# zkonduit/ezkl

Measured on AMD Instinct MI355X. Metric: BN254 G1 MSM pts/s (2^20 points per GPU; NTT 2^22 elems/s in extra), higher is better.
Workload: dtype u32x8 (254-bit modular integer, Montgomery); 1 GPU; configs[1]: standalone 2^20-point BN254 G1 MSM (uniform scalars, try-and-increment bases) + 2^22 scalar-field NTT per GPU; parallelism=points sharded across 1 rank(s); all_gather of 64-B partials + host fold

## Files before the change

ezkl_amd/csrc/msm.hip:

```cpp
#include "common.hpp"
#include <deque>
#include <thread>
#include <chrono>
#include "curve.hpp"
#include "curve29.hpp"
#include "host64.hpp"
#include "msm_plan.hpp"
#include <string.h>

namespace ezkl {

__device__ __forceinline__ uint32_t msm_part_of(uint32_t bucket, uint32_t NP) { return bucket ? 1u + (bucket & (NP - 1u)) : 0u; }
__device__ __forceinline__ uint32_t msm_lane_len(const uint32_t* offsets, uint32_t nb, uint32_t nlanes, uint32_t lmin) {
    const uint32_t l = (uint32_t)(((uint64_t)offsets[nb] + nlanes - 1) / nlanes);
    return l < lmin ? lmin : l;
}

template <class T> __device__ __forceinline__ T* bshift(T* p, size_t bytes) { return reinterpret_cast<T*>(reinterpret_cast<char*>(p) + bytes); }
template <class T> __device__ __forceinline__ const T* bshift(const T* p, size_t bytes) {
    return reinterpret_cast<const T*>(reinterpret_cast<const char*>(p) + bytes);
}
#define BSH(p) p = bshift(p, _bo)
#define BOFF() const size_t _bo = (size_t)blockIdx.z * bstride
struct MsmCols {
// ... 453 lines not shown
            const uint32_t e = beg + t + (uint32_t)q * 512u;
            v[q] = e < end ? entries[e] : make_uint2(0u, 0xffffffffu);
        }
#pragma unroll
        for (int q = 0; q < PER; q++)
            if (v[q].y != 0xffffffffu) atomicAdd(&cnt[v[q].y], 1u);
        __syncthreads();
        msm_bins_scan(cnt, tsum, nbins, p, beg, part_base, true, offsets, buckets);
#pragma unroll
        for (int q = 0; q < PER; q++)
            if (v[q].y != 0xffffffffu) stage[atomicAdd(&cnt[v[q].y], 1u)] = v[q].x;
        __syncthreads();
        for (uint32_t i = t; i < end - beg; i += 512) vals[beg + i] = stage[i];
    } else {
        for (uint32_t e = beg + t; e < end; e += 512) (void)msm_wave_rank(cnt, entries[e].y);
        __syncthreads();
        msm_bins_scan(cnt, tsum, nbins, p, beg, part_base, true, offsets, buckets);
        for (uint32_t e = beg + t; e < end; e += 512) {
            const uint2 v = entries[e];
            vals[beg + msm_wave_rank(cnt, v.y)] = v.x;
        }
    }
}
__device__ __forceinline__ void msm_big_slice(uint32_t beg, uint32_t end, uint32_t& s0, uint32_t& s1, uint32_t bx) {
    const uint32_t chunk = (end - beg + MSM_BIG_BLOCKS - 1) / MSM_BIG_BLOCKS;
    s0 = beg + bx * chunk;
    s1 = s0 + chunk < end ? s0 + chunk : end;
    if (s0 > end) s0 = end;
}
__device__ __forceinline__ void msm_bigsort_count_body(const uint2* entries, const uint32_t* part_base, uint32_t LB, const uint32_t* big_list,
                                                       const uint32_t* big_count, uint32_t* bin_total, uint32_t* block_off, uint32_t* cnt, uint32_t bx,
                                                       uint32_t by, uint32_t rows) {
    const uint32_t t = threadIdx.x, nbins = 1u << LB;
    const uint32_t nbig = big_count[0] < MSM_MAX_BIG ? big_count[0] : MSM_MAX_BIG;
    for (uint32_t y = by; y < nbig; y += rows) {
        const uint32_t p = big_list[y];
        uint32_t s0, s1;
        msm_big_slice(part_base[p + 1], part_base[p + 2], s0, s1, bx);
        for (uint32_t j = t; j < nbins; j += 512) cnt[j] = 0;
        __syncthreads();
        for (uint32_t e = s0 + t; e < s1; e += 512) (void)msm_wave_rank(cnt, entries[e].y);
        __syncthreads();
        for (uint32_t j = t; j < nbins; j += 512)
            block_off[((size_t)y * MSM_BIG_BLOCKS + bx) * nbins + j] = cnt[j] ? atomicAdd(&bin_total[(size_t)y * nbins + j], cnt[j]) : 0u;
        __syncthreads();
    }
}
__global__ __launch_bounds__(512) void msm_bigsort_scatter_kernel(const uint2* entries, const uint32_t* part_base, uint32_t LB, const uint32_t* big_list,
                                                                  const uint32_t* big_count, const uint32_t* bin_total, const uint32_t* block_off,
                                                                  uint32_t* offsets, uint32_t* vals, g1x29_t* buckets, size_t bstride) {
    BOFF(); BSH(entries); BSH(part_base); BSH(big_list); BSH(big_count); BSH(bin_total); BSH(block_off); BSH(offsets); BSH(vals); BSH(buckets);
    __shared__ uint32_t cnt[2048];
    __shared__ uint32_t tsum[512];
    const uint32_t t = threadIdx.x, nbins = 1u << LB;
    const uint32_t nbig = big_count[0] < MSM_MAX_BIG ? big_count[0] : MSM_MAX_BIG;
    for (uint32_t y = blockIdx.y; y < nbig; y += gridDim.y) {
        const uint32_t p = big_list[y], beg = part_base[p + 1];
        uint32_t s0, s1;
        msm_big_slice(beg, part_base[p + 2], s0, s1, blockIdx.x);
        for (uint32_t j = t; j < nbins; j += 512) cnt[j] = bin_total[(size_t)y * nbins + j];
        __syncthreads();
        msm_bins_scan(cnt, tsum, nbins, p, beg, part_base, blockIdx.x == 0, offsets, buckets);
        const uint32_t* mine = block_off + ((size_t)y * MSM_BIG_BLOCKS + blockIdx.x) * nbins;
        for (uint32_t j = t; j < nbins; j += 512) atomicAdd(&cnt[j], mine[j]);
        __syncthreads();
        for (uint32_t e = s0 + t; e < s1; e += 512) {
            const uint2 v = entries[e];
            vals[beg + msm_wave_rank(cnt, v.y)] = v.x;
        }
        __syncthreads();
    }
}

struct MsmRec {
    g1a_t p;
    bool neg;
};
__device__ __forceinline__ MsmRec msm_fetch(const g1a_t* tab, uint32_t v) {
    MsmRec r;
    r.p = ld_g1a(tab + (v & 0x7fffffffu));
    r.neg = (v >> 31) != 0;
    return r;
}
__global__ __launch_bounds__(256, 3) void msm_accumulate_kernel(const g1a_t* tab, const uint32_t* offsets, const uint32_t* vals,
                                                             uint32_t nb, uint32_t nlanes, g1x29_t* buckets, g1x29_t* head, g1x29_t* tail,
                                                             uint32_t* lane_first, uint32_t lmin, size_t bstride) {
    BOFF(); BSH(offsets); BSH(vals); BSH(buckets); BSH(head); BSH(tail); BSH(lane_first);
    const uint32_t t = blockIdx.x * blockDim.x + threadIdx.x;
    const uint32_t total = offsets[nb], L = msm_lane_len(offsets, nb, nlanes, lmin);
    const uint64_t k0w = (uint64_t)t * L;
    if (k0w >= total) return;
    const uint32_t k0 = (uint32_t)k0w;
    const uint32_t k1 = (uint64_t)k0 + L < total ? k0 + L : total;
    uint32_t lo = 0, hi = nb;
    while (hi - lo > 1) {
        uint32_t mid = (lo + hi) >> 1;
        if (offsets[mid] <= k0) lo = mid; else hi = mid;
    }
    uint32_t b = lo, bin_end = offsets[b + 1];
    uint32_t end_next = offsets[b + 2 <= nb ? b + 2 : nb];
    lane_first[t] = b;
    bool started_before = offsets[b] < k0;
    g1x29_t acc = g1x29_identity();
    MsmRec nxt = msm_fetch(tab, vals[k0]);
    uint32_t vn = k0 + 1 < k1 ? vals[k0 + 1] : 0u;
    for (uint32_t k = k0; k < k1; k++) {
        if (k == bin_end) {
            if (started_before) st_g1x29(head + t, acc); else st_g1x29(buckets + b, acc);
            acc.zz = Fq29::zero();
            started_before = false;
            b++;
            bin_end = end_next;
            if (bin_end == k) {
                uint32_t probes = 1;
                while (bin_end == k && probes < 4) { b++; bin_end = offsets[b + 1]; probes++; }
                if (bin_end == k) {
                    uint32_t lo2 = b + 1, hi2 = nb, vhi = total;
                    while (hi2 - lo2 > 1) {
                        const uint32_t mid = (lo2 + hi2) >> 1, vm = offsets[mid];
                        if (vm <= k) lo2 = mid; else { hi2 = mid; vhi = vm; }
                    }
                    b = lo2;
                    bin_end = vhi;
                }
            }
        }
        end_next = offsets[b + 2 <= nb ? b + 2 : nb];
        const MsmRec cur = nxt;
        nxt = msm_fetch(tab, vn);
        vn = k + 2 < k1 ? vals[k + 2] : 0u;
        acc = g1x29_add_mixed(acc, g1a29_unpack(cur.p), cur.neg);
    }
    if (k1 == bin_end) {
        if (started_before) st_g1x29(head + t, acc); else st_g1x29(buckets + b, acc);
    } else {
        if (started_before) st_g1x29(head + t, acc); else st_g1x29(tail + t, acc);
    }
}
EZ_D g1x29_t g1x29_shfl_down(const g1x29_t& p, uint32_t d) {
    g1x29_t r;
    const uint32_t* s = p.x.v;
    uint32_t* o = r.x.v;
#pragma unroll
    for (int k = 0; k < 36; k++) o[k] = __shfl_down(s[k], d);
    return r;
}
__global__ __launch_bounds__(256, 3) void msm_fixup_boundary_tree_kernel(const uint32_t* offsets, uint32_t nb, uint32_t nlanes,
                                                                      const uint32_t* lane_first, const g1x29_t* head, const g1x29_t* tail, g1x29_t* buckets,
                                                                      uint32_t* heavy_list, uint32_t* heavy_count, uint32_t* chunk_list, uint32_t lmin,
                                                                      uint32_t span_heavy, size_t bstride) {
    BOFF(); BSH(offsets); BSH(lane_first); BSH(head); BSH(tail); BSH(buckets); BSH(heavy_list); BSH(heavy_count); BSH(chunk_list);
    const uint32_t t = blockIdx.x * blockDim.x + threadIdx.x + 1;
    const uint32_t lane = threadIdx.x & 63u;
    const uint32_t L = msm_lane_len(offsets, nb, nlanes, lmin);
    const uint64_t k0 = (uint64_t)t * L;
    bool cut = t < nlanes && k0 < offsets[nb];
    uint32_t b = 0, t1 = 0, t2 = 0;
    if (cut) {
        b = lane_first[t];
        const uint32_t beg = offsets[b], end = offsets[b + 1];
        cut = beg < k0;
        t1 = beg / L; t2 = (end - 1) / L;
    }
    if (cut && t2 - t1 > span_heavy) {
        if (t == t1 + 1 && t2 - t1 > MSM_HEAVY_CHUNK) heavy_list[atomicAdd(heavy_count, 1u)] = b;
        if ((t - t1 - 1) % MSM_HEAVY_CHUNK == 0) chunk_list[atomicAdd(heavy_count + 1, 1u)] = t;
        cut = false;
    }
    const uint32_t wave_last = t + (63u - lane);
    const uint32_t run = cut ? (t2 < wave_last ? t2 : wave_last) - t + 1u : 0u;
    uint32_t longest = run;
#pragma unroll
    for (uint32_t o = 32; o > 0; o >>= 1) {
        const uint32_t m = __shfl_xor(longest, o);
        longest = m > longest ? m : longest;
    }
    if (longest == 0) return;
    if (longest <= 2) {
        if (!cut || t != t1 + 1) return;
        g1x29_t acc = g1x29_add(ld_g1x29(tail + t1), ld_g1x29(head + t));
        for (uint32_t u = t + 1; u <= t2; u++) acc = g1x29_add(acc, ld_g1x29(head + u));
        st_g1x29(buckets + b, acc);
        return;
    }
    g1x29_t v = cut ? ld_g1x29(head + t) : g1x29_identity();
    uint32_t have = cut ? 1u : 0u;
#pragma unroll 1
    for (uint32_t d = 1; d < longest; d <<= 1) {
        const g1x29_t w = g1x29_shfl_down(v, d);
        const uint32_t hw = __shfl_down(have, d);
        if (have == d && run > d) {
            v = g1x29_add(v, w);
            have += hw;
        }
    }
    if (!cut || t != t1 + 1) return;
    g1x29_t acc = g1x29_add(ld_g1x29(tail + t1), v);
    for (uint32_t u = t + run; u <= t2; u++) acc = g1x29_add(acc, ld_g1x29(head + u));
    st_g1x29(buckets + b, acc);
}
__global__ __launch_bounds__(256) void msm_fixup_heavy1_kernel(const uint32_t* offsets, uint32_t nb, uint32_t nlanes, const uint32_t* lane_first, g1x29_t* head,
                                                               const g1x29_t* tail, g1x29_t* buckets, const uint32_t* chunk_list, const uint32_t* counts, uint32_t lmin,
                                                               uint32_t coop, size_t bstride) {
    BOFF(); BSH(offsets); BSH(lane_first); BSH(head); BSH(tail); BSH(buckets); BSH(chunk_list); BSH(counts);
    const uint32_t nchunks = counts[1], L = msm_lane_len(offsets, nb, nlanes, lmin);
    const uint32_t wave = threadIdx.x >> 6, lane = threadIdx.x & 63u;
    for (uint32_t ci = blockIdx.x * 4u + wave; ci < nchunks; ci += gridDim.x * 4u) {
        const uint32_t start = chunk_list[ci], b = lane_first[start];
        const uint32_t t2 = (offsets[b + 1] - 1) / L;
        const uint32_t stop = start + MSM_HEAVY_CHUNK - 1 < t2 ? start + MSM_HEAVY_CHUNK - 1 : t2;
        const uint32_t t1 = offsets[b] / L;
        const bool whole = t2 - t1 <= MSM_HEAVY_CHUNK;
        g1x29_t acc = (whole && lane == 63u) ? ld_g1x29(tail + t1) : g1x29_identity();
        for (uint32_t t = start + lane; t <= stop; t += 64) acc = g1x29_add(acc, ld_g1x29(head + t));
        acc = coop ? g1x29_group_sum_coop(acc, 64) : g1x29_group_sum(acc, 64);
        if (lane == 0) st_g1x29(whole ? buckets + b : head + start, acc);
    }
}
__global__ __launch_bounds__(256) void msm_fixup_heavy2_kernel(const uint32_t* offsets, uint32_t nb, uint32_t nlanes, const g1x29_t* head, const g1x29_t* tail,
                                                               const uint32_t* heavy_list, const uint32_t* counts, g1x29_t* buckets, uint32_t lmin, uint32_t coop, size_t bstride) {
    BOFF(); BSH(offsets); BSH(head); BSH(tail); BSH(heavy_list); BSH(counts); BSH(buckets);
    const uint32_t L = msm_lane_len(offsets, nb, nlanes, lmin);
    const uint32_t wave = threadIdx.x >> 6, lane = threadIdx.x & 63u;
    for (uint32_t h = blockIdx.x * 4u + wave; h < counts[0]; h += gridDim.x * 4u) {
        const uint32_t b = heavy_list[h];
        const uint32_t t1 = offsets[b] / L, t2 = (offsets[b + 1] - 1) / L;
        g1x29_t acc = lane == 63u ? ld_g1x29(tail + t1) : g1x29_identity();
        for (uint32_t t = t1 + 1 + lane * MSM_HEAVY_CHUNK; t <= t2; t += 64 * MSM_HEAVY_CHUNK) acc = g1x29_add(acc, ld_g1x29(head + t));
        acc = coop ? g1x29_group_sum_coop(acc, 64) : g1x29_group_sum(acc, 64);
        if (lane == 0) st_g1x29(buckets + b, acc);
    }
}

__global__ __launch_bounds__(256, 2) void msm_reduce1_kernel(const g1x29_t* buckets, ReduceGeom g, g1x29_t* partA, g1x29_t* partT, size_t bstride) {
    BOFF(); BSH(buckets); BSH(partA); BSH(partT);
    const uint32_t idx = blockIdx.x * blockDim.x + threadIdx.x;
    g1x29_t acc = g1x29_identity();
    if (blockIdx.y == 0) {
        if (idx >= (g.GA << g.wA)) return;
        const uint32_t dA = idx & ((1u << g.wA) - 1u), grp = idx >> g.wA;
        for (uint32_t e = 0; e < g.EA; e++) acc = g1x29_add(acc, ld_g1x29(buckets + ((((size_t)grp * g.EA + e) << g.wA) | dA)));
        st_g1x29(partA + (size_t)dA * g.GA + grp, acc);
    } else {
        const uint32_t nT = 1u << (g.wB + g.wC);
        if (idx >= nT * g.GT) return;
        const uint32_t grp = idx % g.GT, t = idx / g.GT;
        for (uint32_t e = 0; e < g.ET; e++) acc = g1x29_add(acc, ld_g1x29(buckets + (((size_t)t << g.wA) | (e * g.GT + grp))));
        st_g1x29(partT + (size_t)t * g.GT + grp, acc);
    }
}
__global__ __launch_bounds__(64) void msm_reduce2_kernel(const g1x29_t* partA, const g1x29_t* partT, ReduceGeom g, g1x29_t* SA, g1x29_t* T, uint32_t lanesA,
                                                         uint32_t lanesT, uint32_t blocksA, uint32_t coop, size_t bstride) {
    BOFF(); BSH(partA); BSH(partT); BSH(SA); BSH(T);
    const bool isA = blockIdx.x < blocksA;
    const uint32_t lanes = isA ? lanesA : lanesT, per = 64 / lanes;
    const uint32_t o = (isA ? blockIdx.x : blockIdx.x - blocksA) * per + threadIdx.x / lanes, j = threadIdx.x % lanes;
    const uint32_t nout = isA ? (1u << g.wA) : (1u << (g.wB + g.wC)), G = isA ? g.GA : g.GT;
    g1x29_t acc = g1x29_identity();
    if (o < nout) {
        const g1x29_t* src = (isA ? partA : partT) + (size_t)o * G;
        for (uint32_t i = j; i < G; i += lanes) acc = g1x29_add(acc, ld_g1x29(src + i));
    }
    acc = (coop && lanes >= 4) ? g1x29_group_sum_coop(acc, lanes) : g1x29_group_sum(acc, lanes);
    if (j == 0 && o < nout) st_g1x29((isA ? SA : T) + o, acc);
}
__global__ __launch_bounds__(256) void msm_planes_kernel(const g1x29_t* SA, const g1x29_t* T, ReduceGeom g, g1x29_t* planes, g1x29_t* planes_host, uint32_t coop,
                                                         size_t bstride) {
    BOFF(); BSH(SA); BSH(T); BSH(planes);
    __shared__ uint4 sh[9 * 4];
    uint32_t id = blockIdx.x, field = 0, j = 0;
    if (id > 0) {
        id -= 1;
        if (id < g.wA) { field = 1; j = id; }
        else if (id < g.wA + g.wB) { field = 2; j = id - g.wA; }
        else { field = 3; j = id - g.wA - g.wB; }
    }
    const uint32_t nA = 1u << g.wA, nT = 1u << (g.wB + g.wC);
    g1x29_t acc = g1x29_identity();
    auto with_bit = [](uint32_t k, uint32_t bit) { return ((k >> bit) << (bit + 1)) | (1u << bit) | (k & ((1u << bit) - 1u)); };
    if (field == 0) {
        for (uint32_t d = threadIdx.x; d < nA; d += 256) acc = g1x29_add(acc, ld_g1x29(SA + d));
    } else if (field == 1) {
        for (uint32_t k = threadIdx.x; k < nA / 2; k += 256) acc = g1x29_add(acc, ld_g1x29(SA + with_bit(k, j)));
    } else {
        const uint32_t sh_bits = field == 2 ? j : g.wB + j;
        for (uint32_t k = threadIdx.x; k < nT / 2; k += 256) acc = g1x29_add(acc, ld_g1x29(T + with_bit(k, sh_bits)));
    }
    acc = (coop & 8u) ? g1x29_block256_sum_coop_full(acc, sh) : coop ? g1x29_block256_sum_coop(acc, sh) : g1x29_block256_sum(acc, sh);
    if (threadIdx.x == 0) {
        const uint32_t ws = field == 1 ? g.wsA : field == 2 ? g.wsB : g.wsC;
        const uint32_t slot = field == 0 ? 0u : 1u + ws + j;
        st_g1x29(planes + slot, acc);
        if (planes_host) st_g1x29(planes_host + (size_t)blockIdx.z * 32 + slot, acc);
    }
}

static int table_build(Ctx* c, hipStream_t st, const Bases* b, bool wait) {
    MsmTable t;
    t.n = b->n;
    t.wp = pick_plan(b->n);
    if ((size_t)t.wp.W * t.n >= ((size_t)1 << 31)) return EZKL_ERR_UNSUPPORTED;
    EZ_HIP(hipMalloc(&t.tab, (size_t)t.wp.W * t.n * sizeof(g1a_t)));
    EZ_HIP(hipMemcpyAsync(t.tab, b->pts, t.n * sizeof(g1a_t), hipMemcpyDeviceToDevice, st));
    for (uint32_t w = 1; w < t.wp.W; w++)
        hipLaunchKernelGGL(msm_precompute_kernel, dim3(cdiv(t.n, 256)), dim3(256), 0, st, t.tab + (size_t)(w - 1) * t.n,
                           t.tab + (size_t)w * t.n, t.n, t.wp.width(w - 1));
    hipLaunchKernelGGL(msm_table_to_r261_kernel, dim3(cdiv((size_t)t.wp.W * t.n, 256)), dim3(256), 0, st, t.tab, (size_t)t.wp.W * t.n);
    EZ_HIP(hipGetLastError());
    EZ_HIP(hipEventCreateWithFlags(&t.ready, hipEventDisableTiming));
    EZ_HIP(hipEventRecord(t.ready, st));
    if (wait) {
        EZ_HIP(hipStreamSynchronize(st));
        t.synced = true;
    }
    g_tables[b] = t;
    return EZKL_OK;
}
static int table_get(Ctx* c, hipStream_t st, const Bases* b, MsmTable** out) {
    auto it = g_tables.find(b);
    if (it == g_tables.end()) {
        int rc = table_build(c, st, b, true);
        if (rc) return rc;
        it = g_tables.find(b);
    }
    if (!it->second.synced) {
        EZ_HIP(hipEventSynchronize(it->second.ready));
        it->second.synced = true;
    }
    *out = &it->second;
    return EZKL_OK;
}
int msm_table_prepare(Ctx* c, const Bases* b) {
    if (g_tables.count(b)) return EZKL_OK;
    if (!g_table_stream) EZ_HIP(hipStreamCreateWithFlags(&g_table_stream, hipStreamNonBlocking));
    return table_build(c, g_table_stream, b, false);
}
void msm_table_drop(const Bases* b) {
    auto it = g_tables.find(b);
    if (it != g_tables.end()) {
        if (it->second.ready) { (void)hipEventSynchronize(it->second.ready); (void)hipEventDestroy(it->second.ready); }
        (void)hipFree(it->second.tab);
        g_tables.erase(it);
    }
}

static int slot_prepare(MsmSlot& sl, size_t bytes, size_t msms = 1) {
    if (!sl.st) {
        EZ_HIP(stream_create_prio(&sl.st, "EZKL_HIP_PRIO_MSM", 0));
        EZ_HIP(hipEventCreateWithFlags(&sl.done, hipEventDisableTiming));
    }
    if (msms > sl.pinned_msms) {
        if (sl.pinned) {
            EZ_HIP(hipStreamSynchronize(sl.st));
            EZ_HIP(hipHostFree(sl.pinned));
            sl.pinned = nullptr;
        }
        EZ_HIP(hipHostMalloc((void**)&sl.pinned, msms * 32 * sizeof(g1x29_t), hipHostMallocDefault));
        EZ_HIP(hipHostGetDevicePointer(&sl.pinned_dev, sl.pinned, 0));
        sl.pinned_msms = msms;
    }
    if (bytes > sl.scratch_bytes) {
        if (sl.scratch) {
            EZ_HIP(hipStreamSynchronize(sl.st));
            EZ_HIP(hipFree(sl.scratch));
            sl.scratch = nullptr;
            sl.scratch_bytes = 0;
        }
        size_t want = bytes + (bytes >> 4);
        EZ_HIP(hipMalloc((void**)&sl.scratch, want));
        sl.scratch_bytes = want;
    }
    return EZKL_OK;
}
static int msm_finish(MsmSlot& sl, void* out_host = nullptr, bool release = true) {
    if (!out_host) out_host = sl.out;
    EZ_HIP(hipEventSynchronize(sl.done));
    for (uint32_t j = 0; j < sl.count; j++) {
        const uint32_t* hp = sl.pinned + (size_t)j * 32 * 36;
        h64::xyzz acc = h64::identity();
        for (int k = (int)sl.bits - 1; k >= 0; k--) {
            acc = h64::dbl(acc);
            acc = h64::add(acc, h64::from_limbs29_point(hp + 36 * (1 + k)));
        }
        acc = h64::add(acc, h64::from_limbs29_point(hp));
        h64::aff r = h64::to_affine(acc);
        memcpy((uint8_t*)out_host + 64 * (size_t)j, &r, 64);
    }
    if (release) sl.busy = false;
    return EZKL_OK;
}

struct MsmKnobs : MsmTuning {
    int group, group_small, group_big;
};
static int msm_env(const char* name, int hi, int dflt) { const char* e = getenv(name); const int v = e ? atoi(e) : 0; return v >= 1 && v <= hi ? v : dflt; }
static MsmKnobs msm_tuning() {
    static const int lmin = msm_env("EZKL_MSM_LMIN", 4096, (int)MSM_LMIN), span = msm_env("EZKL_MSM_SPAN", 4096, (int)MSM_SPAN_HEAVY);
    static const int small = msm_env("EZKL_MSM_GROUP_SMALL", (int)MSM_MAX_GROUP, 6), big = msm_env("EZKL_MSM_GROUP_BIG", (int)MSM_MAX_GROUP, 4);
    MsmKnobs k;
    k.lmin = (uint32_t)lmin; k.span_heavy = (uint32_t)span; k.group_small = small; k.group_big = big;
    k.L_override = (uint32_t)msm_env("EZKL_MSM_L", (1 << 20) - 1, 0);
    const int e = msm_env("EZKL_MSM_E", 1024, 0);
    if (e && (e & (e - 1)) == 0) k.E = (uint32_t)e;
    k.group = msm_env("EZKL_MSM_GROUP", (int)MSM_MAX_GROUP, 0);
    return k;
}
static size_t msm_group_size(bool small_scalars) {
    const MsmKnobs k = msm_tuning();
    return (size_t)(k.group ? k.group : small_scalars ? k.group_small : k.group_big);
}
static int msm_device_init(int& acc_blocks_per_cu) {
    if (acc_blocks_per_cu) return EZKL_OK;
    EZ_HIP(hipFuncSetAttribute((const void*)msm_binsort_kernel, hipFuncAttributeMaxDynamicSharedMemorySize, MSM_BINSORT_LDS));
    EZ_HIP(hipFuncSetAttribute((const void*)msm_partition_kernel, hipFuncAttributeMaxDynamicSharedMemorySize, MSM_PART_LDS));
    EZ_HIP(hipOccupancyMaxActiveBlocksPerMultiprocessor(&acc_blocks_per_cu, msm_accumulate_kernel, 256, 0));
    if (acc_blocks_per_cu < 1) acc_blocks_per_cu = 1;
    return EZKL_OK;
}
static_assert(sizeof(g1x29_t) == MSM_POINT_BYTES, "msm_plan lays the scratch out in points of this size");
static int msm_enqueue(Ctx* c, MsmSlot& sl, hipStream_t st, MsmTable* T, size_t base_offset, const fe_t* const* cols, size_t count, size_t n, bool timed) {
    int rc = EZKL_OK;
    if (count < 1 || count > MSM_MAX_GROUP) return EZKL_ERR_INVALID;
    const unsigned Z = (unsigned)count;
    const MsmKnobs tu = msm_tuning();
    int& acc_blocks_per_cu = msm_state().acc_blocks_per_cu;
    if ((rc = msm_device_init(acc_blocks_per_cu))) return rc;
    const MsmPlan p = msm_plan(n, T->wp, count, c->num_cus, acc_blocks_per_cu, tu);
    const WinPlan wp = T->wp;
    const ReduceGeom rg = p.rg;
    const uint32_t nb = p.nb, LB = p.LB, NP = p.NP, NQ = p.NQ, nlanes = p.nlanes, lmin = tu.lmin, span_heavy = tu.span_heavy;
    const size_t per_block = p.per_block, bstride = p.bstride;
    constexpr uint32_t coop = 7;
    rc = slot_prepare(sl, p.slab_bytes * count, count);
    if (rc) return rc;
    uint8_t* S = sl.scratch;
    MsmCols kcols;
    for (size_t j = 0; j < MSM_MAX_GROUP; j++) kcols.col[j] = cols[j < count ? j : 0];
    auto u32 = [&](size_t o) { return (uint32_t*)(S + o); };
    auto pt = [&](size_t o) { return (g1x29_t*)(S + o); };
    uint2* entries = (uint2*)(S + p.o.ent);
    uint32_t *vals = u32(p.o.vals), *offs = u32(p.o.offs), *pcnt = u32(p.o.pcnt), *pbase = u32(p.o.pbase), *wghist = u32(p.o.wghist);
    uint32_t *heavy = u32(p.o.heavy), *hcnt = u32(p.o.hcnt), *chunks = u32(p.o.chunks), *lfirst = u32(p.o.lfirst);
    uint32_t *bflag = u32(p.o.bflag), *blist = u32(p.o.blist), *btot = u32(p.o.btot), *boff = u32(p.o.boff);
    uint32_t* bcnt = hcnt + 2;
    g1x29_t *bkt = pt(p.o.bkt), *head = pt(p.o.head), *tail = pt(p.o.tail), *planes = pt(p.o.planes);
    g1x29_t *partA = pt(p.o.partA), *partT = pt(p.o.partT), *SA = pt(p.o.SA), *TT = pt(p.o.T);

    hipEvent_t m0 = nullptr, m1 = nullptr, a0 = nullptr, a1 = nullptr;
    bool timed_chain = timed;
    if (timed) {
        const char* tm = getenv("EZKL_HIP_TIMING");
        if (tm && !strcmp(tm, "none")) timed = timed_chain = false;
        else if (tm && !strcmp(tm, "kernel")) timed_chain = false;
    }
    if (timed) {
        if (timed_chain && (rc = ev_pair(c, "msm", &m0, &m1))) return rc;
        if ((rc = ev_pair(c, "msm_accumulate", &a0, &a1))) return rc;
        if (timed_chain) EZ_HIP(hipEventRecord(m0, st));
    }
    hipLaunchKernelGGL(msm_hist_kernel, dim3(p.sgrid, 1, Z), dim3(256), 0, st, kcols, n, per_block, wp, LB, NP, wghist, hcnt,
                       (uint32_t)(p.zero_bytes / 4), bstride);
    hipLaunchKernelGGL(msm_hist_scan_kernel, dim3(cdiv(NQ, MSM_SCAN_COLS), 1, Z), dim3(1024), 0, st, wghist, p.sgrid, NQ, pcnt, bstride);
    hipLaunchKernelGGL(msm_part_scan_kernel, dim3(1, 1, Z), dim3(1024), 0, st, pcnt, NQ, pbase, bflag, blist, bcnt, bstride);
    hipLaunchKernelGGL(msm_partition_kernel, dim3(p.pgrid, 1, Z), dim3((unsigned)per_block), p.part_lds, st, kcols, n, per_block,
                       (uint32_t)p.sgrid, wp, LB, NP, base_offset, T->n, pbase, wghist, pcnt, entries, vals, bstride);
    hipLaunchKernelGGL(msm_binsort_kernel, dim3(NP + MSM_BIG_BLOCKS * MSM_BIG_ROWS, 1, Z), dim3(512), MSM_BINSORT_STAGE * 4, st, entries, pbase, LB, NP, bflag, offs,
                       vals, bkt, blist, bcnt, btot, boff, bstride);
    hipLaunchKernelGGL(msm_bigsort_scatter_kernel, dim3(MSM_BIG_BLOCKS, MSM_BIG_ROWS, Z), dim3(512), 0, st, entries, pbase, LB, blist, bcnt, btot, boff, offs,
                       vals, bkt, bstride);
    if (timed) EZ_HIP(hipEventRecord(a0, st));
    hipLaunchKernelGGL(msm_accumulate_kernel, dim3(cdiv(nlanes, 256), 1, Z), dim3(256), 0, st, T->tab, offs, vals, nb, nlanes, bkt, head, tail,
                       lfirst, lmin, bstride);
    if (timed) EZ_HIP(hipEventRecord(a1, st));
    if (nlanes > 1)
        hipLaunchKernelGGL(msm_fixup_boundary_tree_kernel, dim3(cdiv(nlanes - 1, 256), 1, Z), dim3(256), 0, st, offs, nb, nlanes, lfirst, head, tail, bkt,
                           heavy, hcnt, chunks, lmin, span_heavy, bstride);
    hipLaunchKernelGGL(msm_fixup_heavy1_kernel, dim3(p.cb, 1, Z), dim3(256), 0, st, offs, nb, nlanes, lfirst, head, tail, bkt, chunks, hcnt, lmin, coop & 4u, bstride);
    hipLaunchKernelGGL(msm_fixup_heavy2_kernel, dim3(p.hb, 1, Z), dim3(256), 0, st, offs, nb, nlanes, head, tail, heavy, hcnt, bkt, lmin, coop & 4u, bstride);
    hipLaunchKernelGGL(msm_reduce1_kernel, dim3(p.r1grid, 2, Z), dim3(256), 0, st, bkt, rg, partA, partT, bstride);
    hipLaunchKernelGGL(msm_reduce2_kernel, dim3(p.r2grid, 1, Z), dim3(64), 0, st, partA, partT, rg, SA, TT, p.lanesA, p.lanesT, p.blocksA, coop & 1u, bstride);
    hipLaunchKernelGGL(msm_planes_kernel, dim3(p.nplanes, 1, Z), dim3(256), 0, st, SA, TT, rg, planes, (g1x29_t*)sl.pinned_dev, coop & 10u, bstride);
    EZ_HIP(hipGetLastError());
    if (getenv("EZKL_MSM_DEBUG")) {
        uint32_t hc = 0;
        EZ_HIP(hipMemcpyAsync(&hc, hcnt, 4, hipMemcpyDeviceToHost, st));
        EZ_HIP(hipStreamSynchronize(st));
        fprintf(stderr, "[msm] n=%zu W=%u bits=%u L=%u nlanes=%u heavy=%u\n", n, p.W, p.bits, p.L, nlanes, hc);
    }
    if (timed_chain) EZ_HIP(hipEventRecord(m1, st));
    EZ_HIP(hipEventRecord(sl.done, st));
    sl.bits = p.bits;
    sl.count = (uint32_t)count;
    sl.busy = true;
    return EZKL_OK;
}
static int msm_run_groups(Ctx* c, MsmTable* T, size_t base_offset, const fe_t* const* cols, size_t batch, size_t n, void* out_host,
                          const hipEvent_t* wait_ev, bool small_scalars) {
    const size_t G = msm_group_size(small_scalars);
    static const bool dbg = getenv("EZKL_MSM_DEBUG") != nullptr;
    if (dbg) fprintf(stderr, "[ezkl_hip] msm batch: %zu columns of %zu points, %s scalars, groups of %zu\n", batch, n, small_scalars ? "witness-shaped" : "general", G);
    int rc = EZKL_OK;
    size_t gi = 0;
    for (size_t j0 = 0; j0 < batch && !rc; gi++) {
        size_t cnt = batch - j0 < G ? batch - j0 : G;
        if (wait_ev && j0 > 0) {
            const size_t left = batch - j0;
            cnt = left <= 2 ? 1 : std::min(G, (left + 1) / 2);
        }
        MsmSlot& sl = g_slots[gi % MSM_SLOTS];
        if (sl.busy) rc = msm_finish(sl);
        if (!rc) rc = slot_prepare(sl, 0);
        for (size_t j = 0; wait_ev && j < cnt && !rc; j++)
            if (hipStreamWaitEvent(sl.st, wait_ev[j0 + j], 0) != hipSuccess) rc = EZKL_ERR_HIP;
        if (!rc) {
            sl.out = (uint8_t*)out_host + 64 * j0;
            rc = msm_enqueue(c, sl, sl.st, T, base_offset, cols + j0, cnt, n, false);
        }
        j0 += cnt;
    }
    for (size_t k = 0; k < (size_t)MSM_SLOTS; k++) {
        MsmSlot& sl = g_slots[(gi + k) % MSM_SLOTS];
        if (!sl.busy) continue;
        if (!rc) rc = msm_finish(sl);
        else { (void)hipStreamSynchronize(sl.st); sl.busy = false; }
    }
    return rc;
}

static bool msm_host_timing() { static const bool on = getenv("EZKL_MSM_HOST_TIMING") != nullptr; return on; }
static double msm_now_us() { return std::chrono::duration<double, std::micro>(std::chrono::steady_clock::now().time_since_epoch()).count(); }
static void msm_host_timing_add(size_t n, double t0, double t1, double t2, double t3) {
    static double acc[3] = {0, 0, 0};
    static int calls = 0;
    acc[0] += t1 - t0; acc[1] += t2 - t1; acc[2] += t3 - t2;
    if (++calls % 50 == 0) {
        fprintf(stderr, "[msm host] n=%zu per call: enqueue %.1f us, wait for the GPU %.1f us, host tail %.1f us\n", n, acc[0] / 50, acc[1] / 50, acc[2] / 50);
        acc[0] = acc[1] = acc[2] = 0;
    }
}
static MsmBatch* g_open_batch_fwd();
int msm_run(Ctx* c, hipStream_t st, const Bases* b, size_t base_offset, const fe_t* scalars, size_t n, void* out_host) {
    if (g_open_batch_fwd()) return EZKL_ERR_INVALID;
    if (n == 0) { memset(out_host, 0, 64); return EZKL_OK; }
    MsmTable* T = nullptr;
    int rc = table_get(c, st, b, &T);
    if (rc) return rc;
    MsmSlot& sl = g_slots[0];
    if (sl.busy) return EZKL_ERR_INVALID;
    const bool host_timing = msm_host_timing();
    const double t0 = host_timing ? msm_now_us() : 0;
    if ((rc = msm_enqueue(c, sl, st, T, base_offset, &scalars, 1, n, true))) return rc;
    if (!host_timing) return msm_finish(sl, out_host);
    const double t1 = msm_now_us();
    EZ_HIP(hipEventSynchronize(sl.done));
    const double t2 = msm_now_us();
    rc = msm_finish(sl, out_host);
    msm_host_timing_add(n, t0, t1, t2, msm_now_us());
    return rc;
}

int msm_call_start(Ctx* c, std::unique_lock<std::recursive_mutex>& lk, const Bases* b, size_t base_offset, const fe_t* scalars, size_t n, int* slot_out) {
    if (g_open_batch_fwd() || n == 0) return EZKL_ERR_INVALID;
    MsmTable* T = nullptr;
    int rc = table_get(c, c->stream, b, &T);
    if (rc) return rc;
    int k = -1;
    for (;;) {
        for (int i = 0; i < MSM_CALL_SLOTS && k < 0; i++)
            if (!g_call_claimed[i]) k = i;
        if (k >= 0) break;
        bool all_mine = true;
        for (int i = 0; i < MSM_CALL_SLOTS; i++) all_mine = all_mine && g_call_owner[i] == std::this_thread::get_id();
        if (all_mine) return EZKL_ERR_BUSY;
        lk.unlock();
        std::this_thread::yield();
        lk.lock();
    }
    MsmSlot& sl = g_call_slots[k];
    g_call_claimed[k] = true;
    g_call_finishing[k] = false;
    g_call_owner[k] = std::this_thread::get_id();
    rc = slot_prepare(sl, 0);
    if (!rc) {
        hipError_t e = hipSuccess;
        const hipError_t q = hipStreamQuery(c->stream);
        if (q != hipSuccess) {
            (void)hipGetLastError();
            if (!g_call_order_ev) e = hipEventCreateWithFlags(&g_call_order_ev, hipEventDisableTiming);
            if (e == hipSuccess) e = hipEventRecord(g_call_order_ev, c->stream);
            if (e == hipSuccess) e = hipStreamWaitEvent(sl.st, g_call_order_ev, 0);
        }
        if (e != hipSuccess) rc = set_hip_error(e, "msm_call_start", __FILE__, __LINE__);
    }
    if (!rc) rc = msm_enqueue(c, sl, sl.st, T, base_offset, &scalars, 1, n, true);
    if (rc) { g_call_claimed[k] = false; g_call_owner[k] = std::thread::id(); return rc; }
    *slot_out = k;
    return EZKL_OK;
}
int msm_call_finish(Ctx* c, std::unique_lock<std::recursive_mutex>& lk, int k, void* out_host) {
    (void)c;
    if (k < 0 || k >= MSM_CALL_SLOTS || !g_call_claimed[k] || g_call_finishing[k] || !g_call_slots[k].busy) return EZKL_ERR_INVALID;
    MsmSlot& sl = g_call_slots[k];
    g_call_finishing[k] = true;
    lk.unlock();
    const int rc = msm_finish(sl, out_host, false);
    lk.lock();
    sl.busy = false;
    g_call_finishing[k] = false;
    g_call_claimed[k] = false;
    g_call_owner[k] = std::thread::id();
    return rc;
}
int msm_run_concurrent(Ctx* c, std::unique_lock<std::recursive_mutex>& lk, const Bases* b, size_t base_offset, const fe_t* scalars, size_t n, void* out_host) {
    if (g_open_batch_fwd()) return EZKL_ERR_INVALID;
    if (n == 0) { memset(out_host, 0, 64); return EZKL_OK; }
    int k = -1;
    const bool host_timing = msm_host_timing();
    const double t0 = host_timing ? msm_now_us() : 0;
    int rc = msm_call_start(c, lk, b, base_offset, scalars, n, &k);
    if (rc) return rc;
    if (!host_timing) return msm_call_finish(c, lk, k, out_host);
    const double t1 = msm_now_us();
    (void)hipEventSynchronize(g_call_slots[k].done);
    const double t2 = msm_now_us();
    rc = msm_call_finish(c, lk, k, out_host);
    msm_host_timing_add(n, t0, t1, t2, msm_now_us());
    return rc;
}

int msm_run_batch(Ctx* c, hipStream_t st, const Bases* b, size_t base_offset, const fe_t* const* scalars, size_t batch, size_t n,
                  void* out_host, bool small_scalars) {
// ... 351 lines not shown
```

ezkl_amd/csrc/msm_plan.hpp:

```cpp
#pragma once
#include <cstddef>
#include <cstdint>
#if defined(__HIPCC__) || defined(__HIP__)
#define MSM_HD __host__ __device__
#else
#define MSM_HD
#endif

namespace ezkl {

static constexpr uint32_t MSM_MAX_PART_BITS = 12;
static constexpr uint32_t MSM_SPAN_HEAVY = 16;
static constexpr uint32_t MSM_PART_STAGE = 13312;
static constexpr uint32_t MSM_BINSORT_STAGE = 15360;
static constexpr uint32_t MSM_HEAVY_CHUNK = 256;
static constexpr uint32_t MSM_DIGIT_E = 8;
static constexpr uint32_t MSM_LMIN = 8;
static constexpr uint32_t MSM_MAX_BIG = 64;
static constexpr uint32_t MSM_BIG_BLOCKS = 64;
static constexpr uint32_t MSM_BIG_ROWS = 8;
static constexpr uint32_t MSM_SCAN_COLS = 4;
static constexpr size_t MSM_MAX_GROUP = 16;
static constexpr uint32_t MSM_PART_LDS = 144u << 10;
static constexpr uint32_t MSM_BINSORT_LDS = 96u << 10;
static constexpr size_t MSM_POINT_BYTES = 144;

struct WinPlan {
    uint32_t W, base, rem;
    MSM_HD uint32_t width(uint32_t w) const { return base + (w < rem ? 1u : 0u); }
    MSM_HD uint32_t offset(uint32_t w) const { return w * base + (w < rem ? w : rem); }
    MSM_HD uint32_t cmax() const { return base + (rem ? 1u : 0u); }
};
inline WinPlan pick_plan(size_t n) {
    WinPlan best{0, 0, 0};
    double best_cost = 0;
    for (uint32_t W = 10; W <= 127; W++) {
        WinPlan p{W, 254 / W, 254 % W};
        if (p.cmax() > 23) continue;
        const double cost = (double)n * W + 4.0 * (double)((size_t)1 << (p.cmax() - 1));
        if (!best.W || cost < best_cost) { best = p; best_cost = cost; }
    }
    return best;
}

struct ReduceGeom {
    uint32_t wA, wB, wC;
    uint32_t wsA, wsB, wsC;
    uint32_t EA, GA, ET, GT;
};

struct MsmTuning {
    uint32_t L_override = 0;
    uint32_t E = MSM_DIGIT_E;
    uint32_t lmin = MSM_LMIN;
    uint32_t span_heavy = MSM_SPAN_HEAVY;
};

struct MsmPlan {
    uint32_t W, bits, nb, PB, LB, NP, NQ, L, nlanes;
    size_t npairs, per_block, part_lds;
    unsigned sgrid, pgrid, hb, cb, r1grid, r2grid;
    ReduceGeom rg;
    uint32_t nA, nT, n_partA, n_partT, nplanes, lanesA, lanesT, blocksA;
    struct Off { size_t ent, vals, offs, pcnt, pbase, wghist, heavy, chunks, hcnt, btot, planes, bflag, blist, boff, lfirst, bkt, head, tail, partA, partT, SA, T; } o;
    size_t zero_bytes, slab_bytes, bstride;
};

inline MsmPlan msm_plan(size_t n, WinPlan wp, size_t count, int num_cus, int acc_blocks_per_cu, const MsmTuning& tu) {
    MsmPlan p{};
    auto cdiv = [](size_t a, size_t b) { return (unsigned)((a + b - 1) / b); };
    const uint32_t W = p.W = wp.W, bits = p.bits = wp.cmax() - 1;
    const uint32_t nb = p.nb = 1u << bits;
    const size_t npairs = p.npairs = n * W;
    uint32_t PB = bits < 10 ? bits : 10;
    while (PB < bits && PB < MSM_MAX_PART_BITS && (npairs >> PB) > (size_t)MSM_BINSORT_STAGE * 9 / 10) PB++;
    const uint32_t LB = p.LB = bits - PB, NP = p.NP = 1u << PB;
    const uint32_t NQ = p.NQ = NP + 1;
    p.PB = PB;
    const size_t resident = (size_t)acc_blocks_per_cu * 256 * num_cus;
    const size_t load = npairs >> bits, per_lane = load * 9 / 10 > 40 ? load * 9 / 10 : 40;
    size_t rounds = npairs / (resident * per_lane);
    if (rounds < 1) rounds = 1;
    uint32_t L = (uint32_t)((npairs + resident * rounds - 1) / (resident * rounds));
    if (L < 8) L = 8;
    if (tu.L_override) L = tu.L_override;
    p.L = L;
    const uint32_t nlanes = p.nlanes = cdiv(npairs, L);
    ReduceGeom& rg = p.rg;
    if (LB > 0) {
        rg.wA = LB; rg.wsA = PB;
        rg.wB = (PB + 1) / 2; rg.wsB = 0;
        rg.wC = PB - rg.wB; rg.wsC = rg.wB;
    } else {
        rg.wA = (bits + 2) / 3; rg.wsA = 0;
        rg.wB = (bits - rg.wA + 1) / 2; rg.wsB = rg.wA;
        rg.wC = bits - rg.wA - rg.wB; rg.wsC = rg.wA + rg.wB;
    }
    {
        const uint32_t rows = 1u << (rg.wB + rg.wC), cols = 1u << rg.wA, E = tu.E;
        rg.EA = rows < E ? rows : E; rg.GA = rows / rg.EA;
        rg.ET = cols < E ? cols : E; rg.GT = cols / rg.ET;
    }
    const uint32_t nA = p.nA = 1u << rg.wA, nT = p.nT = 1u << (rg.wB + rg.wC);
    const uint32_t n_partA = p.n_partA = nA * rg.GA, n_partT = p.n_partT = nT * rg.GT;
    const uint32_t nplanes = p.nplanes = 1 + bits;
    size_t per_block = MSM_PART_STAGE / W / 64 * 64;
    {
        const size_t lds_words = MSM_PART_LDS / 4, fixed = 3 * ((size_t)NQ + 1);
        const size_t fit = lds_words > fixed ? (lds_words - fixed) / (2 * (size_t)W) / 64 * 64 : 64;
        if (per_block > fit) per_block = fit;
    }
    if (per_block > 1024) per_block = 1024;
    if (per_block < 64) per_block = 64;
    p.per_block = per_block;
    const unsigned sgrid = p.sgrid = cdiv(n, per_block);
    p.pgrid = sgrid < (unsigned)num_cus ? sgrid : (unsigned)num_cus;
    p.part_lds = (3 * ((size_t)NQ + 1) + 2 * per_block * W) * 4;
    {
        const size_t max_heavy = nlanes / tu.span_heavy + 1, max_chunks = nlanes / MSM_HEAVY_CHUNK + max_heavy;
        const size_t heavy_wgs = (max_heavy + 3) / 4, chunk_wgs = (max_chunks + 3) / 4;
        p.hb = (unsigned)(heavy_wgs < (size_t)num_cus * 4 ? heavy_wgs : (size_t)num_cus * 4);
        p.cb = (unsigned)(chunk_wgs < (size_t)num_cus * 4 ? chunk_wgs : (size_t)num_cus * 4);
    }
    {
        p.r1grid = cdiv(n_partA > n_partT ? n_partA : n_partT, 256);
        auto pow2_le = [](uint32_t x) { uint32_t q = 1; while (q * 2 <= x) q *= 2; return q; };
        uint32_t lanesA = pow2_le(rg.GA < 64 ? rg.GA : 64), lanesT = pow2_le(rg.GT < 64 ? rg.GT : 64);
        auto waves = [&](uint32_t nout, uint32_t lanes) { return cdiv(nout, 64 / lanes); };
        while (waves(nA, lanesA) + waves(nT, lanesT) > (unsigned)num_cus * 4 && (lanesA > 1 || lanesT > 1)) {
            if (lanesT > 1 && waves(nT, lanesT) >= waves(nA, lanesA)) lanesT >>= 1; else if (lanesA > 1) lanesA >>= 1; else lanesT >>= 1;
        }
        p.lanesA = lanesA; p.lanesT = lanesT;
        p.blocksA = waves(nA, lanesA);
        p.r2grid = p.blocksA + waves(nT, lanesT);
    }
    size_t off = 0;
    auto carve = [&](size_t bytes) { size_t o = off; off += (bytes + 255) & ~(size_t)255; return o; };
    MsmPlan::Off& o = p.o;
    o.ent = carve(npairs * 8); o.vals = carve(npairs * 4); o.offs = carve(((size_t)nb + 1) * 4);
    o.pcnt = carve((NQ + 1) * 4); o.pbase = carve((NQ + 1) * 4); o.wghist = carve((size_t)sgrid * NQ * 4);
    o.heavy = carve((size_t)nb * 4); o.chunks = carve(((size_t)nlanes + 1) * 4);
    const size_t nbins = (size_t)1 << LB;
    o.hcnt = carve(256); o.btot = carve(MSM_MAX_BIG * nbins * 4); o.planes = carve((size_t)nplanes * MSM_POINT_BYTES);
    p.zero_bytes = off - o.hcnt;
    o.bflag = carve((size_t)NP * 4); o.blist = carve(MSM_MAX_BIG * 4); o.boff = carve((size_t)MSM_MAX_BIG * MSM_BIG_BLOCKS * nbins * 4);
    o.lfirst = carve((size_t)nlanes * 4);
    o.bkt = carve((size_t)nb * MSM_POINT_BYTES);
    o.head = carve((size_t)nlanes * MSM_POINT_BYTES); o.tail = carve((size_t)nlanes * MSM_POINT_BYTES);
    o.partA = carve((size_t)n_partA * MSM_POINT_BYTES); o.partT = carve((size_t)n_partT * MSM_POINT_BYTES);
    o.SA = carve((size_t)nA * MSM_POINT_BYTES); o.T = carve((size_t)nT * MSM_POINT_BYTES);
    p.slab_bytes = off;
    p.bstride = count > 1 ? off : 0;
    return p;
}

}
```

Baseline: 831.0 million pts/s.

## Fuse heavy-bucket fixup passes with atomic tickets and prefetch boundary loads

Merges the two heavy-bucket fixup kernels into one launch. Each chunk bumps a per-bucket atomic ticket stored in the chunk list, and the last chunk to finish performs the final cross-chunk reduction after acquire/release fences. The boundary tree kernel now loads head, tail and lane_first up front, unconditionally, so their latency overlaps the offset lookups. The coop mask also widens from 7 to 15, which turns on an extra cooperative path in the planes kernel. This saves a launch and a dependency boundary, at the cost of extra atomics, speculative loads and ticket slots that share storage in the chunk list.

```diff
diff --git a/ezkl_amd/csrc/msm.hip b/ezkl_amd/csrc/msm.hip
--- a/ezkl_amd/csrc/msm.hip
+++ b/ezkl_amd/csrc/msm.hip
@@ -629,21 +629,28 @@
     BOFF(); BSH(offsets); BSH(lane_first); BSH(head); BSH(tail); BSH(buckets); BSH(heavy_list); BSH(heavy_count); BSH(chunk_list);
     const uint32_t t = blockIdx.x * blockDim.x + threadIdx.x + 1;
     const uint32_t lane = threadIdx.x & 63u;
+    const uint32_t tc = t < nlanes ? t : nlanes - 1u, tp = tc ? tc - 1u : 0u;
+    const uint32_t b = lane_first[tc];
+    const g1x29_t hd = ld_g1x29(head + tc);
+    const g1x29_t tl = ld_g1x29(tail + tp);
     const uint32_t L = msm_lane_len(offsets, nb, nlanes, lmin);
     const uint64_t k0 = (uint64_t)t * L;
     bool cut = t < nlanes && k0 < offsets[nb];
-    uint32_t b = 0, t1 = 0, t2 = 0;
+    uint32_t t1 = 0, t2 = 0;
     if (cut) {
-        b = lane_first[t];
         const uint32_t beg = offsets[b], end = offsets[b + 1];
         cut = beg < k0;
         t1 = beg / L; t2 = (end - 1) / L;
     }
     if (cut && t2 - t1 > span_heavy) {
-        if (t == t1 + 1 && t2 - t1 > MSM_HEAVY_CHUNK) heavy_list[atomicAdd(heavy_count, 1u)] = b;
+        if (t == t1 + 1 && t2 - t1 > MSM_HEAVY_CHUNK) {
+            heavy_list[atomicAdd(heavy_count, 1u)] = b;
+            chunk_list[msm_heavy_ticket_slot(nlanes, t)] = 0;
+        }
         if ((t - t1 - 1) % MSM_HEAVY_CHUNK == 0) chunk_list[atomicAdd(heavy_count + 1, 1u)] = t;
         cut = false;
     }
+    const bool first = cut && t == t1 + 1;
     const uint32_t wave_last = t + (63u - lane);
     const uint32_t run = cut ? (t2 < wave_last ? t2 : wave_last) - t + 1u : 0u;
     uint32_t longest = run;
@@ -654,13 +661,13 @@
     }
     if (longest == 0) return;
     if (longest <= 2) {
-        if (!cut || t != t1 + 1) return;
-        g1x29_t acc = g1x29_add(ld_g1x29(tail + t1), ld_g1x29(head + t));
+        if (!first) return;
+        g1x29_t acc = g1x29_add(tl, hd);
         for (uint32_t u = t + 1; u <= t2; u++) acc = g1x29_add(acc, ld_g1x29(head + u));
         st_g1x29(buckets + b, acc);
         return;
     }
-    g1x29_t v = cut ? ld_g1x29(head + t) : g1x29_identity();
+    g1x29_t v = cut ? hd : g1x29_identity();
     uint32_t have = cut ? 1u : 0u;
 #pragma unroll 1
     for (uint32_t d = 1; d < longest; d <<= 1) {
@@ -671,8 +678,9 @@
             have += hw;
         }
     }
-    if (!cut || t != t1 + 1) return;
-    g1x29_t acc = g1x29_add(ld_g1x29(tail + t1), v);
+    __builtin_amdgcn_s_waitcnt(0xc07f);
+    if (!first) return;
+    g1x29_t acc = g1x29_add(ld_g1x29(tail + (t - 1u)), v);
     for (uint32_t u = t + run; u <= t2; u++) acc = g1x29_add(acc, ld_g1x29(head + u));
     st_g1x29(buckets + b, acc);
 }
@@ -703,6 +711,39 @@
         const uint32_t b = heavy_list[h];
         const uint32_t t1 = offsets[b] / L, t2 = (offsets[b + 1] - 1) / L;
         g1x29_t acc = lane == 63u ? ld_g1x29(tail + t1) : g1x29_identity();
+        for (uint32_t t = t1 + 1 + lane * MSM_HEAVY_CHUNK; t <= t2; t += 64 * MSM_HEAVY_CHUNK) acc = g1x29_add(acc, ld_g1x29(head + t));
+        acc = coop ? g1x29_group_sum_coop(acc, 64) : g1x29_group_sum(acc, 64);
+        if (lane == 0) st_g1x29(buckets + b, acc);
+    }
+}
+__global__ __launch_bounds__(256) void msm_fixup_heavy_kernel(const uint32_t* offsets, uint32_t nb, uint32_t nlanes, const uint32_t* lane_first, g1x29_t* head,
+                                                              const g1x29_t* tail, g1x29_t* buckets, uint32_t* chunk_list, const uint32_t* counts, uint32_t lmin,
+                                                              uint32_t coop, size_t bstride) {
+    BOFF(); BSH(offsets); BSH(lane_first); BSH(head); BSH(tail); BSH(buckets); BSH(chunk_list); BSH(counts);
+    const uint32_t nchunks = counts[1];
+    if (nchunks == 0) return;
+    const uint32_t L = msm_lane_len(offsets, nb, nlanes, lmin);
+    const uint32_t wave = threadIdx.x >> 6, lane = threadIdx.x & 63u;
+    for (uint32_t ci = blockIdx.x * 4u + wave; ci < nchunks; ci += gridDim.x * 4u) {
+        const uint32_t start = chunk_list[ci], b = lane_first[start];
+        const uint32_t t2 = (offsets[b + 1] - 1) / L;
+        const uint32_t stop = start + MSM_HEAVY_CHUNK - 1 < t2 ? start + MSM_HEAVY_CHUNK - 1 : t2;
+        const uint32_t t1 = offsets[b] / L;
+        const bool whole = t2 - t1 <= MSM_HEAVY_CHUNK;
+        g1x29_t acc = (whole && lane == 63u) ? ld_g1x29(tail + t1) : g1x29_identity();
+        for (uint32_t t = start + lane; t <= stop; t += 64) acc = g1x29_add(acc, ld_g1x29(head + t));
+        acc = coop ? g1x29_group_sum_coop(acc, 64) : g1x29_group_sum(acc, 64);
+        if (lane == 0) st_g1x29(whole ? buckets + b : head + start, acc);
+        if (whole) continue;
+        uint32_t done = 0;
+        if (lane == 0) {
+            __builtin_amdgcn_fence(__ATOMIC_RELEASE, "agent", "global");
+            done = atomicAdd(&chunk_list[msm_heavy_ticket_slot(nlanes, t1 + 1)], 1u);
+        }
+        done = (uint32_t)__builtin_amdgcn_readfirstlane((int)done);
+        if (done + 1u != (t2 - t1 + MSM_HEAVY_CHUNK - 1) / MSM_HEAVY_CHUNK) continue;
+        __builtin_amdgcn_fence(__ATOMIC_ACQUIRE, "agent", "global");
+        acc = lane == 63u ? ld_g1x29(tail + t1) : g1x29_identity();
         for (uint32_t t = t1 + 1 + lane * MSM_HEAVY_CHUNK; t <= t2; t += 64 * MSM_HEAVY_CHUNK) acc = g1x29_add(acc, ld_g1x29(head + t));
         acc = coop ? g1x29_group_sum_coop(acc, 64) : g1x29_group_sum(acc, 64);
         if (lane == 0) st_g1x29(buckets + b, acc);
@@ -869,6 +910,7 @@
 
 struct MsmKnobs : MsmTuning {
     int group, group_small, group_big;
+    bool heavy_split;
 };
 static int msm_env(const char* name, int hi, int dflt) { const char* e = getenv(name); const int v = e ? atoi(e) : 0; return v >= 1 && v <= hi ? v : dflt; }
 static MsmKnobs msm_tuning() {
@@ -880,6 +922,7 @@
     const int e = msm_env("EZKL_MSM_E", 1024, 0);
     if (e && (e & (e - 1)) == 0) k.E = (uint32_t)e;
     k.group = msm_env("EZKL_MSM_GROUP", (int)MSM_MAX_GROUP, 0);
+    k.heavy_split = msm_env("EZKL_MSM_HEAVY_SPLIT", 1, 0) != 0;
     return k;
 }
 static size_t msm_group_size(bool small_scalars) {
@@ -907,7 +950,7 @@
     const ReduceGeom rg = p.rg;
     const uint32_t nb = p.nb, LB = p.LB, NP = p.NP, NQ = p.NQ, nlanes = p.nlanes, lmin = tu.lmin, span_heavy = tu.span_heavy;
     const size_t per_block = p.per_block, bstride = p.bstride;
-    constexpr uint32_t coop = 7;
+    constexpr uint32_t coop = 15;
     rc = slot_prepare(sl, p.slab_bytes * count, count);
     if (rc) return rc;
     uint8_t* S = sl.scratch;
@@ -952,8 +995,12 @@
     if (nlanes > 1)
         hipLaunchKernelGGL(msm_fixup_boundary_tree_kernel, dim3(cdiv(nlanes - 1, 256), 1, Z), dim3(256), 0, st, offs, nb, nlanes, lfirst, head, tail, bkt,
                            heavy, hcnt, chunks, lmin, span_heavy, bstride);
-    hipLaunchKernelGGL(msm_fixup_heavy1_kernel, dim3(p.cb, 1, Z), dim3(256), 0, st, offs, nb, nlanes, lfirst, head, tail, bkt, chunks, hcnt, lmin, coop & 4u, bstride);
-    hipLaunchKernelGGL(msm_fixup_heavy2_kernel, dim3(p.hb, 1, Z), dim3(256), 0, st, offs, nb, nlanes, head, tail, heavy, hcnt, bkt, lmin, coop & 4u, bstride);
+    if (tu.heavy_split) {
+        hipLaunchKernelGGL(msm_fixup_heavy1_kernel, dim3(p.cb, 1, Z), dim3(256), 0, st, offs, nb, nlanes, lfirst, head, tail, bkt, chunks, hcnt, lmin, coop & 4u, bstride);
+        hipLaunchKernelGGL(msm_fixup_heavy2_kernel, dim3(p.hb, 1, Z), dim3(256), 0, st, offs, nb, nlanes, head, tail, heavy, hcnt, bkt, lmin, coop & 4u, bstride);
+    } else {
+        hipLaunchKernelGGL(msm_fixup_heavy_kernel, dim3(p.cb, 1, Z), dim3(256), 0, st, offs, nb, nlanes, lfirst, head, tail, bkt, chunks, hcnt, lmin, coop & 4u, bstride);
+    }
     hipLaunchKernelGGL(msm_reduce1_kernel, dim3(p.r1grid, 2, Z), dim3(256), 0, st, bkt, rg, partA, partT, bstride);
     hipLaunchKernelGGL(msm_reduce2_kernel, dim3(p.r2grid, 1, Z), dim3(64), 0, st, partA, partT, rg, SA, TT, p.lanesA, p.lanesT, p.blocksA, coop & 1u, bstride);
     hipLaunchKernelGGL(msm_planes_kernel, dim3(p.nplanes, 1, Z), dim3(256), 0, st, SA, TT, rg, planes, (g1x29_t*)sl.pinned_dev, coop & 10u, bstride);
diff --git a/ezkl_amd/csrc/msm_plan.hpp b/ezkl_amd/csrc/msm_plan.hpp
--- a/ezkl_amd/csrc/msm_plan.hpp
+++ b/ezkl_amd/csrc/msm_plan.hpp
@@ -42,6 +42,8 @@
     }
     return best;
 }
+
+MSM_HD inline uint32_t msm_heavy_ticket_slot(uint32_t nlanes, uint32_t first_boundary) { return nlanes / 2 + first_boundary / 2; }
 
 struct ReduceGeom {
     uint32_t wA, wB, wC;
```

Measured after the change: 826.6 million pts/s. Within noise of the previous version (-0.5%).
